# hellojialee/Improved-Body-Parts

Hardware: AMD Instinct MI355X
Metric: fps_512_infer (higher is better)
Workload: dtype bf16; 1 GPU; model=4-stage IMHN @512x512, mode=infer, global_batch=4, input=512, parallelism=dp1

## Files before the change

### improved_body_parts_amd/ops/csrc/bindings.cpp

```cpp
#include <torch/extension.h>

using torch::Tensor;

std::vector<int64_t> bn_v8_geometry(int64_t M, int64_t C);
std::vector<Tensor> bn_stats(const Tensor& x_mc, int64_t C);
std::vector<Tensor> bn_finalize(
    const Tensor& sums, const Tensor& sumsq, int64_t M, const Tensor& gamma,
    const Tensor& beta, const c10::optional<Tensor>& running_mean,
    const c10::optional<Tensor>& running_var,
    const c10::optional<Tensor>& num_batches, double momentum, double eps);
std::vector<Tensor> bn_stats_finalize(
    const Tensor& x_mc, int64_t C, const Tensor& gamma, const Tensor& beta,
    const c10::optional<Tensor>& running_mean,
    const c10::optional<Tensor>& running_var,
    const c10::optional<Tensor>& num_batches, double momentum, double eps);
Tensor bn_act_fwd(const Tensor& x, const Tensor& scale, const Tensor& shift,
                  const c10::optional<Tensor>& residual, double slope, bool act);
std::vector<Tensor> bn_act_bwd(const Tensor& dy, const Tensor& y, const Tensor& x,
                               const c10::optional<Tensor>& mean,
                               const c10::optional<Tensor>& invstd,
                               double slope, bool act, bool need_xhat, int64_t C);
Tensor bn_act_bwd_apply(const Tensor& dpre, const Tensor& x, const Tensor& mean,
                        const Tensor& invstd, const Tensor& gamma,
                        const c10::optional<Tensor>& sum_dpre,
                        const c10::optional<Tensor>& sum_dxhat, int64_t C);

std::vector<Tensor> maxpool2x2_fwd(const Tensor& x, int64_t N, int64_t H,
                                   int64_t W, int64_t C);
Tensor maxpool2x2_bwd(const Tensor& dy, const Tensor& arg, int64_t N, int64_t H,
                      int64_t W, int64_t C);
Tensor upsample2x_fwd(const Tensor& x, int64_t N, int64_t H, int64_t W, int64_t C);
Tensor upsample2x_bwd(const Tensor& dy, int64_t N, int64_t H, int64_t W, int64_t C);
Tensor se_reduce(const Tensor& a, const c10::optional<Tensor>& b, int64_t N,
                 int64_t HW, int64_t C);
Tensor se_scale(const Tensor& x, const Tensor& s, const c10::optional<Tensor>& addc,
                int64_t N, int64_t HW, int64_t C);
Tensor se_gate(const Tensor& pooled, const Tensor& w1, const Tensor& b1,
               const Tensor& w2, const Tensor& b2, double slope,
               double pool_scale);
std::vector<Tensor> se_layer_grouped(const std::vector<Tensor>& xs,
                                     const std::vector<Tensor>& w1s,
                                     const std::vector<Tensor>& b1s,
                                     const std::vector<Tensor>& w2s,
                                     const std::vector<Tensor>& b2s,
                                     double slope);

Tensor focal_l2_fwd(const Tensor& pred, const Tensor& gt, const Tensor& mask,
                    int64_t heat_start, int64_t bkg_start, int64_t gamma,
                    double mtw, double ktw, double alpha, double beta);
Tensor focal_l2_bwd(const Tensor& pred, const Tensor& gt, const Tensor& mask,
                    const Tensor& stack_gscale, int64_t heat_start,
                    int64_t bkg_start, int64_t gamma, double mtw, double ktw,
                    double alpha, double beta);

Tensor conv_mfma_fwd(const Tensor& x, const Tensor& w_packed,
                     const std::vector<int64_t>& geom,
                     const c10::optional<Tensor>& scale,
                     const c10::optional<Tensor>& shift,
                     const c10::optional<Tensor>& residual, bool act,
                     const c10::optional<Tensor>& residual_post,
                     const c10::optional<Tensor>& residual_post2,
                     const c10::optional<Tensor>& x2);

std::vector<Tensor> conv_mfma_fwd_grouped(
    const std::vector<Tensor>& xs, const std::vector<Tensor>& ws_packed,
    const std::vector<std::vector<int64_t>>& geom,
    const std::vector<c10::optional<Tensor>>& scales,
    const std::vector<c10::optional<Tensor>>& shifts,
    const std::vector<c10::optional<Tensor>>& residuals,
    const std::vector<bool>& acts,
    const std::vector<c10::optional<Tensor>>& residual_posts,
    const std::vector<c10::optional<Tensor>>& residual_post2s);

std::vector<int64_t> conv_mfma_tile_plan(int64_t M, int64_t Cout, int64_t K);
std::vector<int64_t> conv_mfma_conv_plan(const Tensor& x,
                                         const Tensor& w_packed,
                                         const std::vector<int64_t>& geom);

void pack_conv_weight(const Tensor& w, Tensor& fwd_pack,
                      const c10::optional<Tensor>& dgrad_pack);

void pack_upfold_weight(const Tensor& w, Tensor& out);
void pack_cat_weight(const Tensor& wa, const Tensor& wb,
                     const c10::optional<Tensor>& scale_a,
                     const c10::optional<Tensor>& scale_b,
                     const c10::optional<Tensor>& shift_a,
                     const c10::optional<Tensor>& shift_b, Tensor& out,
                     Tensor& shift_out);
Tensor conv_mfma_upfold_fwd(const Tensor& x_low, const Tensor& packs,
                            const std::vector<int64_t>& geom,
                            const c10::optional<Tensor>& scale,
                            const c10::optional<Tensor>& shift, bool act,
                            const c10::optional<Tensor>& residual_post,
                            const c10::optional<Tensor>& residual_post2);
std::vector<int64_t> conv_mfma_upfold_plan(int64_t M_low, int64_t Cout,
                                           int64_t Cin);

Tensor conv_mfma_wgrad(const Tensor& x, const Tensor& dy, int64_t N, int64_t H,
                       int64_t W, int64_t Cin, int64_t Cout, int64_t KH,
                       int64_t KW, int64_t stride, int64_t pad_h, int64_t pad_w,
                       int64_t dil_h, int64_t dil_w, int64_t Ho, int64_t Wo);
std::vector<int64_t> conv_wgrad_plan(int64_t M, int64_t Cin, int64_t Cout,
                                     int64_t KH, int64_t KW);
Tensor tr16_probe();

void fused_sgd(const Tensor& chunk_table, double lr, double momentum,
               double weight_decay, int64_t dtype_tag);

Tensor heatmap_gt(const Tensor& joints, const c10::optional<Tensor>& mask_all,
                  const Tensor& limb_pairs, int64_t h, int64_t w,
                  int64_t stride, int64_t heat_start, int64_t bkg_start,
                  int64_t num_layers, double sigma, double paf_sigma,
                  double keypoint_thre, double limb_thre, double paf_thre);

Tensor peaks_batched(const Tensor& maps, int64_t heat_layers, double thre,
                     int64_t radius, int64_t max_peaks);

Tensor limb_scores(const Tensor& paf, const Tensor& peaks, const Tensor& cand_idx,
                   int64_t mid_num, double thre2);
std::vector<Tensor> peaks_canonical(const Tensor& buf, int64_t n_parts);
std::vector<Tensor> limb_match(const Tensor& maps, const Tensor& peaks,
                               const Tensor& offsets, const Tensor& limbs,
                               int64_t first_limb_plane, int64_t mid_num,
                               double thre2, double connect_ration,
                               int64_t max_part);

std::vector<Tensor> people_assemble(const Tensor& peaks, const Tensor& offsets,
                                    const Tensor& rows, const Tensor& counts,
                                    const Tensor& limbs, const Tensor& dt_gt,
                                    double len_rate, double connection_tole,
                                    int64_t remove_recon, int64_t max_people);

void ensemble_merge(const Tensor& src, const Tensor& chan_main,
                    const Tensor& chan_flip, const Tensor& ystart,
                    const Tensor& yw, const Tensor& xstart, const Tensor& xw,
                    Tensor& out, double scale, bool accumulate, int64_t cb,
                    int64_t wr, int64_t wc, int64_t span);

std::vector<Tensor> augment_warp(const Tensor& packed, const Tensor& desc,
                                 int64_t H, int64_t W, int64_t stride,
                                 bool bf16_out);

PYBIND11_MODULE(TORCH_EXTENSION_NAME, m) {
  m.def("bn_v8_geometry", &bn_v8_geometry,
        "debug: [cpb, rpb, rows, grid_y] of the bf16 v8 stats/reduce launch",
        py::arg("M"), py::arg("C"));
  m.def("bn_stats", &bn_stats, "per-channel sum/sumsq of an [M][C] view");
  m.def("bn_finalize", &bn_finalize,
        "mean/invstd/scale/shift epilogue over given (possibly all-reduced) sums");
  m.def("bn_stats_finalize", &bn_stats_finalize,
        "stats + mean/invstd/scale/shift epilogue (+ running-stat update)");
  m.def("bn_act_fwd", &bn_act_fwd, "fused scale/shift (+res) (+leaky)");
  m.def("bn_act_bwd", &bn_act_bwd, "dpre + per-channel reductions");
  m.def("bn_act_bwd_apply", &bn_act_bwd_apply, "BN backward input grad");
  m.def("maxpool2x2_fwd", &maxpool2x2_fwd);
  m.def("maxpool2x2_bwd", &maxpool2x2_bwd);
  m.def("upsample2x_fwd", &upsample2x_fwd);
  m.def("upsample2x_bwd", &upsample2x_bwd);
  m.def("se_reduce", &se_reduce);
  m.def("se_scale", &se_scale);
  m.def("se_gate", &se_gate, "fused GAP-gate: sigmoid(W2@leaky(W1@p+b1)+b2)",
        py::arg("pooled"), py::arg("w1"), py::arg("b1"), py::arg("w2"),
        py::arg("b2"), py::arg("slope"), py::arg("pool_scale") = 1.0);
  m.def("se_layer_grouped", &se_layer_grouped,
        "inference SE layers of independent maps: one launch per stage");
  m.def("focal_l2_fwd", &focal_l2_fwd);
  m.def("focal_l2_bwd", &focal_l2_bwd);
  m.def("conv_mfma_fwd", &conv_mfma_fwd, "MFMA implicit-GEMM conv forward",
        py::arg("x"), py::arg("w_packed"), py::arg("geom"),
        py::arg("scale") = c10::nullopt, py::arg("shift") = c10::nullopt,
        py::arg("residual") = c10::nullopt, py::arg("act") = false,
        py::arg("residual_post") = c10::nullopt,
        py::arg("residual_post2") = c10::nullopt,
        py::arg("x2") = c10::nullopt);
  m.def("conv_mfma_fwd_grouped", &conv_mfma_fwd_grouped,
        "independent MFMA convs in one grouped launch per 8 (+ one combine)",
        py::arg("xs"), py::arg("ws_packed"), py::arg("geom"),
        py::arg("scales"), py::arg("shifts"), py::arg("residuals"),
        py::arg("acts"), py::arg("residual_posts"),
        py::arg("residual_post2s"));
  m.def("conv_mfma_tile_plan", &conv_mfma_tile_plan,
        "debug: [BM, BN, splitk, deep] planned for GEMM extents (M, Cout, K)",
        py::arg("M"), py::arg("Cout"), py::arg("K"));
  m.def("conv_mfma_conv_plan", &conv_mfma_conv_plan,
        "debug: [BM, BN, splitk, deep, gather] planned for conv_mfma_fwd(x, "
        "w_packed, geom); gather 1 = tap-uniform, 0 = generic",
        py::arg("x"), py::arg("w_packed"), py::arg("geom"));
  m.def("pack_conv_weight", &pack_conv_weight,
        "fwd + dgrad weight packs in one kernel",
        py::arg("w"), py::arg("fwd_pack"), py::arg("dgrad_pack") = c10::nullopt);
  m.def("pack_upfold_weight", &pack_upfold_weight,
        "3x3 weight -> four folded 2x2 packs [4][Cout][4*Cin] (nearest-x2 "
        "upsample folded into the conv)",
        py::arg("w"), py::arg("out"));
  m.def("pack_cat_weight", &pack_cat_weight,
        "two 1x1 weights (+ per-channel scales, shifts) -> one [Cout][Ca+Cb] "
        "pack and the fused shift of a two-source 1x1 conv",
        py::arg("wa"), py::arg("wb"), py::arg("scale_a"), py::arg("scale_b"),
        py::arg("shift_a"), py::arg("shift_b"), py::arg("out"),
        py::arg("shift_out"));
  m.def("conv_mfma_upfold_fwd", &conv_mfma_upfold_fwd,
        "conv3x3(nearest_x2(x_low)) + epilogue as four parity 2x2 convs in "
        "one grouped launch",
        py::arg("x_low"), py::arg("packs"), py::arg("geom"),
        py::arg("scale") = c10::nullopt, py::arg("shift") = c10::nullopt,
        py::arg("act") = false, py::arg("residual_post") = c10::nullopt,
        py::arg("residual_post2") = c10::nullopt);
  m.def("conv_mfma_upfold_plan", &conv_mfma_upfold_plan,
        "debug: [BM, BN, splitk, deep] shared by the four parities of an "
        "upfold conv over M_low low-resolution pixels",
        py::arg("M_low"), py::arg("Cout"), py::arg("Cin"));
  m.def("conv_mfma_wgrad", &conv_mfma_wgrad,
        "MFMA implicit-GEMM conv weight gradient (tr16 LDS transpose)");
  m.def("conv_wgrad_plan", &conv_wgrad_plan,
        "debug: [TKD, TCO, waves, elem, kd_cb, chunks, chunk_len, tree group "
        "counts...] planned for a weight gradient with M = N*Ho*Wo",
        py::arg("M"), py::arg("Cin"), py::arg("Cout"), py::arg("KH"),
        py::arg("KW"));
  m.def("tr16_probe", &tr16_probe,
        "debug: ds_read_b64_tr_b16 delivery-map probe");
  m.def("fused_sgd", &fused_sgd);
  m.def("heatmap_gt", &heatmap_gt, "on-device GT heatmap/PAF generation",
        py::arg("joints"), py::arg("mask_all"), py::arg("limb_pairs"),
        py::arg("h"), py::arg("w"), py::arg("stride"), py::arg("heat_start"),
        py::arg("bkg_start"), py::arg("num_layers"), py::arg("sigma"),
        py::arg("paf_sigma"), py::arg("keypoint_thre"), py::arg("limb_thre"),
        py::arg("paf_thre"));
  m.def("limb_scores", &limb_scores);
  m.def("peaks_canonical", &peaks_canonical,
        "peaks_batched buffer -> rows in (channel, y, x) order + channel offsets",
        py::arg("buf"), py::arg("n_parts"));
  m.def("limb_match", &limb_match,
        "per (image, limb): score, filter and greedily match all nA x nB segments",
        py::arg("maps"), py::arg("peaks"), py::arg("offsets"), py::arg("limbs"),
        py::arg("first_limb_plane"), py::arg("mid_num"), py::arg("thre2"),
        py::arg("connect_ration"), py::arg("max_part"));
  m.def("people_assemble", &people_assemble,
        "per image: greedy person assembly over limb_match rows + COCO keypoints",
        py::arg("peaks"), py::arg("offsets"), py::arg("rows"), py::arg("counts"),
        py::arg("limbs"), py::arg("dt_gt"), py::arg("len_rate"),
        py::arg("connection_tole"), py::arg("remove_recon"),
        py::arg("max_people"));
  m.def("peaks_batched", &peaks_batched,
        "fused NMS + centroid refinement over a planar batch, per-image counters",
        py::arg("maps"), py::arg("heat_layers"), py::arg("thre"),
        py::arg("radius"), py::arg("max_peaks"));
  m.def("ensemble_merge", &ensemble_merge,
        "flip-merge + composed bicubic resample of the low-res network output",
        py::arg("src"), py::arg("chan_main"), py::arg("chan_flip"),
        py::arg("ystart"), py::arg("yw"), py::arg("xstart"), py::arg("xw"),
        py::arg("out"), py::arg("scale"), py::arg("accumulate"), py::arg("cb"),
        py::arg("wr"), py::arg("wc"), py::arg("span"));
  m.def("augment_warp", &augment_warp,
        "batched affine warp of ragged uint8 records -> [image NHWC, "
        "mask_miss, mask_all on the stride grid]",
        py::arg("packed"), py::arg("desc"), py::arg("H"), py::arg("W"),
        py::arg("stride"), py::arg("bf16_out"));
}
```

### improved_body_parts_amd/ops/csrc/conv_mfma.hip

```cpp
#include <torch/extension.h>
#include <ATen/hip/HIPContext.h>
#include <algorithm>
#include <type_traits>
#include <vector>
#include "common.h"
#include "conv_params.h"
#include "conv_plan.h"

namespace ibp {

typedef short short8 __attribute__((ext_vector_type(8)));
typedef float floatx4 __attribute__((ext_vector_type(4)));
typedef float floatx2 __attribute__((ext_vector_type(2)));
typedef unsigned short ushortv8 __attribute__((ext_vector_type(8)));
typedef unsigned short ushortv4 __attribute__((ext_vector_type(4)));

__device__ __forceinline__ int lds_off(int row, int k) {
  return row * BK + (k ^ ((row & 7) << 3));
}

template <int BM, int BN, bool DEEP, bool UP, bool CAT, bool TU,
          typename Params>
__device__ __forceinline__ void conv_mfma_body(const Params& p,
                                               const int bid,
                                               unsigned short* lds_a,
                                               unsigned short* lds_b) {
  const int tid = threadIdx.x;
  const int lane = tid & 63;
  const int wave = tid >> 6;

  const int ntiles_n = (p.Cout + BN - 1) / BN;
  const int sk = bid % p.splitk;
  const int tile = bid / p.splitk;
  const int mt = tile / ntiles_n;
  const int nt = tile % ntiles_n;
  const long long m0 = (long long)mt * BM;
  const int n0 = nt * BN;

  constexpr int WROWS = (BM == 128) ? ((BN == 128) ? 2 : 4) : 2;
  constexpr int WCOLS = 4 / WROWS;
  constexpr int WM = BM / WROWS;
  constexpr int WN = BN / WCOLS;
  constexpr int AFRAG = WM / 16;
  constexpr int BFRAG = WN / 16;
  const int wm = (WCOLS == 1) ? wave : (wave >> 1);
  const int wn = (WCOLS == 1) ? 0 : (wave & 1);
  const int row_base = wm * WM;
  const int col_base = wn * WN;

  floatx4 acc[AFRAG][BFRAG];
  #pragma unroll
  for (int i = 0; i < AFRAG; ++i)
    #pragma unroll
    for (int j = 0; j < BFRAG; ++j) acc[i][j] = floatx4{0.f, 0.f, 0.f, 0.f};

  constexpr int A_ELEMS = BM * BK / 256;
  constexpr int B_ELEMS = BN * BK / 256;
  constexpr int TPR_A = BK / A_ELEMS;
  constexpr int TPR_B = BK / B_ELEMS;
  const int a_row = tid / TPR_A;
  const int a_off = (tid % TPR_A) * A_ELEMS;
  const int b_row = tid / TPR_B;
  const int b_off = (tid % TPR_B) * B_ELEMS;

  const long long a_m = m0 + a_row;
  int a_n = 0, a_ho = 0, a_wo = 0;
  bool a_valid_row = a_m < p.M;
  if (a_valid_row && p.m32) {
    unsigned t = (unsigned)a_m;
    a_wo = (int)(t % (unsigned)p.Wo); t /= (unsigned)p.Wo;
    a_ho = (int)(t % (unsigned)p.Ho);
    a_n = (int)(t / (unsigned)p.Ho);
  } else if (a_valid_row) {
    long long t = a_m;
    a_wo = (int)(t % p.Wo); t /= p.Wo;
    a_ho = (int)(t % p.Ho);
    a_n = (int)(t / p.Ho);
  }
  const int hi_base = a_ho * p.stride - p.pad_h;
  const int wi_base = a_wo * p.stride - p.pad_w;

  const int nk_total = (p.K + BK - 1) / BK;
  const int nk_chunk = (nk_total + p.splitk - 1) / p.splitk;
  const int k_begin = sk * nk_chunk;
  const int nk = min(nk_chunk, nk_total - k_begin);
  if (nk <= 0) return;

  unsigned short a_reg0[A_ELEMS];
  unsigned short b_reg0[B_ELEMS];
  unsigned short a_reg1[A_ELEMS];
  unsigned short b_reg1[B_ELEMS];

  int t_kk = k_begin * BK + a_off;
  int t_ci = 0, t_kh = 0, t_kw = 0;
  if constexpr (!CAT) {
    const int t_f = t_kk / p.Cin;
    t_ci = t_kk - t_f * p.Cin;
    t_kh = t_f / p.KW;
    t_kw = t_f - t_kh * p.KW;
  }
  auto tap_advance = [&](int& ci, int& kh, int& kw, int step) {
// ... 409 lines not shown
      }
      #pragma unroll
      for (int i = 0; i < AFRAG; ++i) {
        const long long m = m0 + row_base + i * 16 + epix;
        if (m >= p.M) continue;
        const long long lin = m * p.Cout + col;
        if (p.splitk > 1) {
          *reinterpret_cast<floatx4*>(ws_slice + lin) = acc[i][j];
          continue;
        }
        const long long idx = out_idx(i, col, lin);
        *reinterpret_cast<ushortv4*>(p.y + idx) =
            finish(acc[i][j], idx, sc, sh);
      }
      continue;
    }
    if (p.pair_epi) {
      #pragma unroll
      for (int r = 0; r < 4; r += 2) {
        if (col + r >= p.Cout) continue;
        const float sc0 = p.scale ? p.scale[col + r] : 1.f;
        const float sc1 = p.scale ? p.scale[col + r + 1] : 1.f;
        const float sh0 = p.shift ? p.shift[col + r] : 0.f;
        const float sh1 = p.shift ? p.shift[col + r + 1] : 0.f;
        #pragma unroll
        for (int i = 0; i < AFRAG; ++i) {
          const long long m = m0 + row_base + i * 16 + epix;
          if (m >= p.M) continue;
          const long long lin = m * p.Cout + col + r;
          if (p.splitk > 1) {
            *reinterpret_cast<floatx2*>(ws_slice + lin) =
                floatx2{acc[i][j][r], acc[i][j][r + 1]};
            continue;
          }
          const long long idx = out_idx(i, col + r, lin);
          unsigned r0 = 0, r1 = 0, r2 = 0;
          if (p.res) r0 = *reinterpret_cast<const unsigned*>(p.res + idx);
          if (p.res_post)
            r1 = *reinterpret_cast<const unsigned*>(p.res_post + idx);
          if (p.res_post2)
            r2 = *reinterpret_cast<const unsigned*>(p.res_post2 + idx);
          float v0 = acc[i][j][r] * sc0 + sh0;
          float v1 = acc[i][j][r + 1] * sc1 + sh1;
          if (p.res) {
            v0 += us2f((unsigned short)r0); v1 += us2f((unsigned short)(r0 >> 16));
          }
          if (p.act) { v0 = leaky(v0, 0.01f); v1 = leaky(v1, 0.01f); }
          if (p.res_post) {
            v0 += us2f((unsigned short)r1); v1 += us2f((unsigned short)(r1 >> 16));
          }
          if (p.res_post2) {
            v0 += us2f((unsigned short)r2); v1 += us2f((unsigned short)(r2 >> 16));
          }
          *reinterpret_cast<unsigned*>(p.y + idx) =
              (unsigned)f2us(v0) | ((unsigned)f2us(v1) << 16);
        }
      }
      continue;
    }
    #pragma unroll
    for (int r = 0; r < 4; ++r) {
      if (col + r >= p.Cout) continue;
      const float sc = p.scale ? p.scale[col + r] : 1.f;
      const float sh = p.shift ? p.shift[col + r] : 0.f;
      #pragma unroll
      for (int i = 0; i < AFRAG; ++i) {
        const long long m = m0 + row_base + i * 16 + epix;
        if (m >= p.M) continue;
        const long long lin = m * p.Cout + col + r;
        if (p.splitk > 1) {
          ws_slice[lin] = acc[i][j][r];
          continue;
        }
        const long long idx = out_idx(i, col + r, lin);
        float v = acc[i][j][r] * sc + sh;
        if (p.res) v += us2f(p.res[idx]);
        if (p.act) v = leaky(v, 0.01f);
        if (p.res_post) v += us2f(p.res_post[idx]);
        if (p.res_post2) v += us2f(p.res_post2[idx]);
        p.y[idx] = f2us(v);
      }
    }
  }
}

template <int BM, int BN, bool DEEP = false, bool CAT = false, bool TU = false>
__global__ __launch_bounds__(256, 2) void conv_mfma_kernel(ConvParams p) {
  static_assert(!(CAT && TU), "the two-source conv keeps its own gather");
  __shared__ unsigned short lds_a[2 * BM * BK];
  __shared__ unsigned short lds_b[2 * BN * BK];
  conv_mfma_body<BM, BN, DEEP, false, CAT, TU>(p, blockIdx.x, lds_a, lds_b);
}

template <bool UP>
__global__ __launch_bounds__(256, 2) void conv_mfma_grouped_kernel(
    ConvGroupParams g) {
  __shared__ __attribute__((aligned(16))) unsigned short lds[4 * 128 * BK];
  const int gb = blockIdx.x;
  int pi = 0, base = 0, cfg = g.cfg[0];
  #pragma unroll
  for (int i = 0; i < kMaxGroup - 1; ++i) {
    if (i + 1 < g.n && gb >= g.block_end[i]) {
      pi = i + 1;
      base = g.block_end[i];
      cfg = g.cfg[i + 1];
    }
  }
  typedef __attribute__((address_space(4))) const char* kernarg_bytes;
  kernarg_bytes ka = (kernarg_bytes)__builtin_amdgcn_kernarg_segment_ptr();
  typedef __attribute__((address_space(4))) const ConvParams* kernarg_params;
  const auto& p = *(kernarg_params)(ka + offsetof(ConvGroupParams, p) +
                                    (size_t)pi * sizeof(ConvParams));
  const int bid = gb - base;
  #define IBP_BODY(BM_, BN_, DEEP_, TU_)                                     \
    conv_mfma_body<BM_, BN_, DEEP_, UP, false, TU_>(p, bid, lds,            \
                                                    lds + 2 * BM_ * BK)
  switch (cfg | (p.gather ? 8 : 0)) {
    case tile_cfg(128, 128, false): IBP_BODY(128, 128, false, false); break;
    case tile_cfg(128, 128, true): IBP_BODY(128, 128, true, false); break;
    case tile_cfg(128, 64, false): IBP_BODY(128, 64, false, false); break;
    case tile_cfg(128, 64, true): IBP_BODY(128, 64, true, false); break;
    case tile_cfg(64, 64, false): IBP_BODY(64, 64, false, false); break;
    case tile_cfg(64, 64, true): IBP_BODY(64, 64, true, false); break;
    case tile_cfg(32, 64, false): IBP_BODY(32, 64, false, false); break;
    case tile_cfg(32, 64, true): IBP_BODY(32, 64, true, false); break;
    case 8 | tile_cfg(128, 128, false): IBP_BODY(128, 128, false, true); break;
    case 8 | tile_cfg(128, 128, true): IBP_BODY(128, 128, true, true); break;
    case 8 | tile_cfg(128, 64, false): IBP_BODY(128, 64, false, true); break;
    case 8 | tile_cfg(128, 64, true): IBP_BODY(128, 64, true, true); break;
    case 8 | tile_cfg(64, 64, false): IBP_BODY(64, 64, false, true); break;
    case 8 | tile_cfg(64, 64, true): IBP_BODY(64, 64, true, true); break;
    case 8 | tile_cfg(32, 64, false): IBP_BODY(32, 64, false, true); break;
    default: IBP_BODY(32, 64, true, true); break;
  }
  #undef IBP_BODY
}

static_assert(std::is_same<decltype(&conv_mfma_grouped_kernel<false>),
                           void (*)(ConvGroupParams)>::value &&
                  std::is_same<decltype(&conv_mfma_grouped_kernel<true>),
                               void (*)(ConvGroupParams)>::value,
              "conv_mfma_grouped_kernel must take the table as its only "
              "argument: it is read at kernarg offset 0");

__device__ __forceinline__ float combine_one(float v, float sc, float sh,
                                             bool has_scale, bool has_res,
                                             float r0, int act, bool has_rp,
                                             float r1, bool has_rp2, float r2) {
  if (has_scale) v = v * sc + sh;
  if (has_res) v += r0;
  if (act) v = leaky(v, 0.01f);
  if (has_rp) v += r1;
  if (has_rp2) v += r2;
  return v;
}

__device__ __forceinline__ long long scatter_pixel(unsigned m,
                                                   const OutScatter& s) {
  const unsigned j = m % (unsigned)s.Wo; m /= (unsigned)s.Wo;
  const unsigned i = m % (unsigned)s.Ho;
  const unsigned n = m / (unsigned)s.Ho;
  return ((long long)n * (2 * s.Ho) + 2 * i + s.py) * (2 * s.Wo) + 2 * j + s.px;
}

template <bool VEC, bool UP>
__device__ __forceinline__ void splitk_combine_body(
    const float* __restrict__ ws, unsigned short* __restrict__ y,
    const float* __restrict__ scale, const float* __restrict__ shift,
    const unsigned short* __restrict__ res,
    const unsigned short* __restrict__ res_post,
    const unsigned short* __restrict__ res_post2, long long total, int C,
    int act, int splitk, int bid, int nblocks, const OutScatter& os) {
  if constexpr (VEC) {
    const int C8 = C >> 3;
    const long long groups = total >> 3;
    const long long step = (long long)nblocks * blockDim.x;
    long long g = bid * (long long)blockDim.x + threadIdx.x;
    if (g >= groups) return;
    int c8 = (int)(g % C8);
    const int cstep = (int)(step % C8);
    unsigned row = UP ? (unsigned)(g / C8) : 0u;
    const unsigned rstep = UP ? (unsigned)(step / C8) : 0u;
    for (; g < groups; g += step) {
      const long long w = g << 3;
      const long long i = UP ? scatter_pixel(row, os) * C + c8 * 8 : w;
      floatx4 lo = floatx4{0.f, 0.f, 0.f, 0.f}, hi = lo;
      for (int s = 0; s < splitk; ++s) {
        const float* src = ws + (long long)s * total + w;
        lo += *reinterpret_cast<const floatx4*>(src);
        hi += *reinterpret_cast<const floatx4*>(src + 4);
      }
      floatx4 sc_lo = lo, sc_hi = lo, sh_lo = lo, sh_hi = lo;
      if (scale) {
        sc_lo = *reinterpret_cast<const floatx4*>(scale + c8 * 8);
        sc_hi = *reinterpret_cast<const floatx4*>(scale + c8 * 8 + 4);
        sh_lo = *reinterpret_cast<const floatx4*>(shift + c8 * 8);
        sh_hi = *reinterpret_cast<const floatx4*>(shift + c8 * 8 + 4);
      }
      ushortv8 r0 = ushortv8{0, 0, 0, 0, 0, 0, 0, 0}, r1 = r0, r2 = r0;
      if (res) r0 = *reinterpret_cast<const ushortv8*>(res + i);
      if (res_post) r1 = *reinterpret_cast<const ushortv8*>(res_post + i);
      if (res_post2) r2 = *reinterpret_cast<const ushortv8*>(res_post2 + i);
      ushortv8 out;
      #pragma unroll
      for (int e = 0; e < 4; ++e) {
        out[e] = f2us(combine_one(lo[e], sc_lo[e], sh_lo[e], scale != nullptr,
                                  res != nullptr, us2f(r0[e]), act,
                                  res_post != nullptr, us2f(r1[e]),
                                  res_post2 != nullptr, us2f(r2[e])));
        out[e + 4] = f2us(combine_one(
            hi[e], sc_hi[e], sh_hi[e], scale != nullptr, res != nullptr,
            us2f(r0[e + 4]), act, res_post != nullptr, us2f(r1[e + 4]),
            res_post2 != nullptr, us2f(r2[e + 4])));
      }
      *reinterpret_cast<ushortv8*>(y + i) = out;
      c8 += cstep;
      if (c8 >= C8) c8 -= C8;
      if constexpr (UP) {
        row += rstep;
        if (c8 < cstep) ++row;
      }
    }
  } else {
    for (long long w = bid * (long long)blockDim.x + threadIdx.x;
         w < total; w += (long long)nblocks * blockDim.x) {
      int c = (int)(w % C);
      const long long i =
          UP ? scatter_pixel((unsigned)(w / C), os) * C + c : w;
      float v = 0.f;
      for (int s = 0; s < splitk; ++s) v += ws[(long long)s * total + w];
      v = combine_one(v, scale ? scale[c] : 1.f, scale ? shift[c] : 0.f,
                      scale != nullptr, res != nullptr,
                      res ? us2f(res[i]) : 0.f, act, res_post != nullptr,
                      res_post ? us2f(res_post[i]) : 0.f,
                      res_post2 != nullptr,
                      res_post2 ? us2f(res_post2[i]) : 0.f);
      y[i] = f2us(v);
    }
// ... 207 lines not shown
                         const OptTensor& residual_post2) {
  TORCH_CHECK(x.is_cuda() && x.scalar_type() == at::ScalarType::BFloat16,
              "conv_mfma: x must be a bf16 device tensor");
  TORCH_CHECK(w_packed.is_contiguous(), "conv_mfma: pack must be contiguous");
  TORCH_CHECK(geom.size() == 15, "conv_mfma: geom needs 15 ints");
  ConvProblem q;
  ibp::ConvParams& p = q.p;
  int* const row[15] = {&p.N, &p.H, &p.W, &p.Cin, &p.Cout, &p.KH, &p.KW,
                        &p.stride, &p.pad_h, &p.pad_w, &p.dil_h, &p.dil_w,
                        &p.Ho, &p.Wo, &p.zs};
  for (int i = 0; i < 15; ++i) *row[i] = (int)geom[i];
  p.x = reinterpret_cast<const unsigned short*>(x.data_ptr());
  p.w = reinterpret_cast<const unsigned short*>(w_packed.data_ptr());
  p.scale = scale.has_value() ? scale->data_ptr<float>() : nullptr;
  p.shift = shift.has_value() ? shift->data_ptr<float>() : nullptr;
  p.res = bf16_ptr(residual);
  p.res_post = bf16_ptr(residual_post);
  p.res_post2 = bf16_ptr(residual_post2);
  p.act = act ? 1 : 0;
  return q;
}

void set_second_source(ConvProblem& q, const Tensor& x, const Tensor& x2,
                       const Tensor& w_packed) {
  ibp::ConvParams& p = q.p;
  TORCH_CHECK(x2.is_cuda() && x2.device() == x.device() &&
              x2.scalar_type() == at::ScalarType::BFloat16 && x2.dim() == 4 &&
              x2.is_contiguous(at::MemoryFormat::ChannelsLast) &&
              x2.size(0) == p.N && x2.size(2) == p.H && x2.size(3) == p.W,
              "conv_mfma: x2 must be channels_last bf16 [N, Cin2, H, W]");
  TORCH_CHECK(x.dim() == 4 &&
              x.is_contiguous(at::MemoryFormat::ChannelsLast) &&
              x.size(0) == p.N && x.size(1) == p.Cin && x.size(2) == p.H &&
              x.size(3) == p.W,
              "conv_mfma: with x2, x must be channels_last [N, Cin, H, W]");
  p.Cin2 = (int)x2.size(1);
  p.x2 = reinterpret_cast<const unsigned short*>(x2.data_ptr());
  TORCH_CHECK(w_packed.numel() == (int64_t)p.Cout * (p.Cin + p.Cin2),
              "conv_mfma: two-source pack must be [Cout][Cin + Cin2]");
}

Tensor alloc_output(ConvProblem& q, const Tensor& x) {
  Tensor y = torch::empty({q.p.N, q.p.Ho, q.p.Wo, q.p.Cout}, x.options());
  q.p.y = reinterpret_cast<unsigned short*>(y.data_ptr());
  return y;
}

template <class F>
void with_flag(bool flag, F&& f) {
  if (flag) f(std::true_type{});
  else f(std::false_type{});
}

template <class F>
void with_tile(const ConvPlan& plan, F&& f) {
  using i128 = std::integral_constant<int, 128>;
  using i64 = std::integral_constant<int, 64>;
  using i32 = std::integral_constant<int, 32>;
  with_flag(plan.t.deep, [&](auto deep) {
    if (plan.t.BM == 128 && plan.t.BN == 128) f(i128{}, i128{}, deep);
    else if (plan.t.BM == 128) f(i128{}, i64{}, deep);
    else if (plan.t.BM == 64) f(i64{}, i64{}, deep);
    else f(i32{}, i64{}, deep);
  });
}

void launch_single(const ConvPlan& plan, hipStream_t stream) {
  const ibp::ConvParams& p = plan.p;
  TORCH_CHECK(!p.up, "upfold plans launch through the grouped kernel");
  with_tile(plan, [&](auto bm, auto bn, auto deep) {
    TORCH_CHECK(!(p.Cin2 != 0 && p.gather != 0));
    with_flag(p.Cin2 != 0, [&](auto cat) {
      with_flag(p.gather != 0, [&](auto tu) {
        if constexpr (!(decltype(cat)::value && decltype(tu)::value))
          hipLaunchKernelGGL(
              (ibp::conv_mfma_kernel<decltype(bm)::value, decltype(bn)::value,
                                     decltype(deep)::value,
                                     decltype(cat)::value,
                                     decltype(tu)::value>),
              dim3(plan.nblocks), dim3(256), 0, stream, p);
      });
    });
  });
  if (p.splitk > 1)
    with_flag(plan.vec_combine, [&](auto vec) {
      hipLaunchKernelGGL(ibp::splitk_combine_kernel<decltype(vec)::value>,
                         dim3(ibp::combine_blocks(plan)), dim3(256), 0, stream,
                         p.ws, p.y, p.scale, p.shift, p.res, p.res_post,
                         p.res_post2, (long long)p.M * p.Cout, p.Cout, p.act,
                         p.splitk);
    });
}

void launch_group(const ibp::GroupPlan& gp, hipStream_t stream) {
  with_flag(gp.up, [&](auto up) {
    hipLaunchKernelGGL(ibp::conv_mfma_grouped_kernel<decltype(up)::value>,
                       dim3(gp.blocks), dim3(256), 0, stream, gp.g);
    if (gp.cg.n > 0)
      hipLaunchKernelGGL(
          ibp::splitk_combine_grouped_kernel<decltype(up)::value>,
          dim3(gp.cblocks), dim3(256), 0, stream, gp.cg);
  });
}

void run_plans(std::vector<ConvPlan>& plans, hipStream_t stream,
               const at::TensorOptions& f32) {
  std::vector<Tensor> keep;
  auto workspace = [&](long long elems) -> float* {
    if (elems <= 0) return nullptr;
    keep.push_back(torch::empty({elems}, f32));
    return keep.back().data_ptr<float>();
  };
  for (size_t first = 0; first < plans.size(); first += ibp::kMaxGroup) {
    const size_t last =
        std::min(plans.size(), first + (size_t)ibp::kMaxGroup);
    ConvPlan& head = plans[first];
    if (last - first == 1 && !head.p.up) {
      if (head.ws_elems > 0) ibp::set_workspace(head, workspace(head.ws_elems));
      launch_single(head, stream);
    } else {
      float* ws = workspace(ibp::group_workspace(plans, first, last));
      launch_group(ibp::assemble_group(plans, first, last, ws), stream);
    }
  }
}

}

Tensor conv_mfma_fwd(const Tensor& x, const Tensor& w_packed,
                     const std::vector<int64_t>& geom, const OptTensor& scale,
                     const OptTensor& shift, const OptTensor& residual,
                     bool act, const OptTensor& residual_post,
                     const OptTensor& residual_post2, const OptTensor& x2) {
  ConvProblem q = make_problem(x, w_packed, geom, scale, shift, residual, act,
                               residual_post, residual_post2);
  if (x2.has_value()) set_second_source(q, x, *x2, w_packed);
  Tensor y = alloc_output(q, x);
  std::vector<ConvPlan> plans{ibp::plan_conv(q)};
  run_plans(plans, at::hip::getCurrentHIPStream().stream(),
            x.options().dtype(torch::kFloat32));
  return y;
}

std::vector<Tensor> conv_mfma_fwd_grouped(
    const std::vector<Tensor>& xs, const std::vector<Tensor>& ws_packed,
    const std::vector<std::vector<int64_t>>& geom,
    const std::vector<OptTensor>& scales, const std::vector<OptTensor>& shifts,
    const std::vector<OptTensor>& residuals, const std::vector<bool>& acts,
    const std::vector<OptTensor>& residual_posts,
    const std::vector<OptTensor>& residual_post2s) {
  const size_t n = xs.size();
  TORCH_CHECK(n > 0 && ws_packed.size() == n && geom.size() == n &&
              scales.size() == n && shifts.size() == n &&
              residuals.size() == n && acts.size() == n &&
              residual_posts.size() == n && residual_post2s.size() == n,
              "conv_mfma_fwd_grouped: argument lists differ in length");
  std::vector<ConvPlan> plans;
  std::vector<Tensor> ys;
  plans.reserve(n);
  ys.reserve(n);
  for (size_t i = 0; i < n; ++i) {
    TORCH_CHECK(xs[i].device() == xs[0].device());
    ConvProblem q = make_problem(xs[i], ws_packed[i], geom[i], scales[i],
                                 shifts[i], residuals[i], acts[i],
                                 residual_posts[i], residual_post2s[i]);
    ys.push_back(alloc_output(q, xs[i]));
    plans.push_back(ibp::plan_conv(q));
  }
  run_plans(plans, at::hip::getCurrentHIPStream().stream(),
            xs[0].options().dtype(torch::kFloat32));
  return ys;
}

Tensor conv_mfma_upfold_fwd(const Tensor& x_low, const Tensor& packs,
                            const std::vector<int64_t>& geom,
                            const OptTensor& scale, const OptTensor& shift,
                            bool act, const OptTensor& residual_post,
                            const OptTensor& residual_post2) {
  ConvProblem q = make_problem(x_low, packs, geom, scale, shift, c10::nullopt,
                               act, residual_post, residual_post2);
  ibp::ConvParams& p = q.p;
  const int64_t N = p.N, H = p.H, W = p.W, Cin = p.Cin, Cout = p.Cout;
  TORCH_CHECK(p.KH == 3 && p.KW == 3 && p.stride == 1 && p.pad_h == 1 &&
              p.pad_w == 1 && p.dil_h == 1 && p.dil_w == 1 && p.zs == 1 &&
              p.Ho == 2 * H && p.Wo == 2 * W,
              "conv_mfma_upfold_fwd: geom must be a 3x3 stride-1 pad-1 conv "
              "with Ho x Wo = 2H x 2W");
  TORCH_CHECK(x_low.is_contiguous() && x_low.numel() == N * H * W * Cin,
              "conv_mfma_upfold_fwd: x_low must be contiguous [N][H][W][Cin]");
  TORCH_CHECK(packs.is_cuda() &&
              packs.scalar_type() == at::ScalarType::BFloat16 &&
              packs.numel() == 16 * Cout * Cin,
              "conv_mfma_upfold_fwd: packs must be bf16 [4][Cout][4*Cin]");
  for (const auto* r : {&residual_post, &residual_post2})
    TORCH_CHECK(!r->has_value() || (*r)->numel() == 4 * N * H * W * Cout,
                "conv_mfma_upfold_fwd: residuals must be bf16 "
                "[N][2H][2W][Cout]");
  Tensor y = alloc_output(q, x_low);
  p.KH = p.KW = 2;
  p.Ho = p.H;
  p.Wo = p.W;
  p.up = 1;
  q.tile = ibp::plan_upfold_tile(N * H * W, p.Cout, p.Cin);
  std::vector<ConvPlan> plans;
  plans.reserve(4);
  for (int par = 0; par < 4; ++par) {
    p.py = par >> 1;
    p.px = par & 1;
    p.pad_h = 1 - p.py;
    p.pad_w = 1 - p.px;
    p.w = reinterpret_cast<const unsigned short*>(packs.data_ptr()) +
          (long long)par * Cout * 4 * Cin;
    plans.push_back(ibp::plan_conv(q));
  }
  run_plans(plans, at::hip::getCurrentHIPStream().stream(),
            x_low.options().dtype(torch::kFloat32));
  return y;
}

std::vector<int64_t> conv_mfma_tile_plan(int64_t M, int64_t Cout, int64_t K) {
  const ibp::TilePlan t = ibp::plan_tile(M, (int)Cout, (int)K);
  return {t.BM, t.BN, t.splitk, t.deep ? 1 : 0};
}

std::vector<int64_t> conv_mfma_conv_plan(const Tensor& x,
                                         const Tensor& w_packed,
                                         const std::vector<int64_t>& geom) {
  const ConvProblem q =
      make_problem(x, w_packed, geom, c10::nullopt, c10::nullopt, c10::nullopt,
                   false, c10::nullopt, c10::nullopt);
  const ConvPlan plan = ibp::plan_conv(q);
  return {plan.t.BM, plan.t.BN, plan.p.splitk, plan.t.deep ? 1 : 0,
          plan.p.gather};
}

std::vector<int64_t> conv_mfma_upfold_plan(int64_t M_low, int64_t Cout,
                                           int64_t Cin) {
  const ibp::TilePlan t = ibp::plan_upfold_tile(M_low, (int)Cout, (int)Cin);
  return {t.BM, t.BN, t.splitk, t.deep ? 1 : 0};
}
```

### improved_body_parts_amd/ops/csrc/conv_params.h

```cpp
#pragma once

#include <cstddef>
#include <type_traits>

namespace ibp {

constexpr int BK = 64;

struct ConvParams {
  const unsigned short* x;
  const unsigned short* w;
  unsigned short* y;
  const float* scale;
  const float* shift;
  const unsigned short* res;
  const unsigned short* res_post;
  const unsigned short* res_post2;
  int N, H, W, Cin, Cout, KH, KW;
  int stride, pad_h, pad_w, dil_h, dil_w, Ho, Wo;
  int zs;
  long long M;
  int K;
  int n_mtiles;
  int act;
  int splitk;
  float* ws;
  int vec_epi;
  int pair_epi;
  int m32;
  int up, py, px;
  int Cin2;
  const unsigned short* x2;
  int gather;
};

constexpr long long kGatherMaxBytes = 0x7fffffffLL;
constexpr unsigned kGatherOob = 0x80000000u;

constexpr int kMaxGroup = 8;

struct ConvGroupParams {
  ConvParams p[kMaxGroup];
  int block_end[kMaxGroup];
  int cfg[kMaxGroup];
  int n;
};

constexpr int tile_cfg(int BM, int BN, bool deep) {
  return ((BM == 128 ? (BN == 128 ? 0 : 1) : (BM == 64 ? 2 : 3)) << 1) |
         (deep ? 1 : 0);
}

static_assert(offsetof(ConvGroupParams, p) == 0 &&
                  std::is_standard_layout<ConvGroupParams>::value &&
                  std::is_trivially_copyable<ConvGroupParams>::value &&
                  sizeof(ConvParams) % alignof(ConvParams) == 0 &&
                  sizeof(ConvGroupParams) <= 4096,
              "ConvGroupParams layout: problem array first, within the "
              "kernel-argument limit");

struct OutScatter {
  int up, py, px, Ho, Wo;
};

struct CombineProblem {
  const float* ws;
  unsigned short* y;
  const float* scale;
  const float* shift;
  const unsigned short* res;
  const unsigned short* res_post;
  const unsigned short* res_post2;
  long long total;
  int C, act, splitk, vec;
  OutScatter os;
};

struct CombineGroupParams {
  CombineProblem c[kMaxGroup];
  int block_end[kMaxGroup];
  int n;
};

}
```

### improved_body_parts_amd/ops/csrc/conv_plan.h

```cpp
#pragma once

#include <algorithm>
#include <cstdint>
#include <cstdlib>
#include <optional>
#include <stdexcept>
#include <string>
#include <vector>

#include "conv_params.h"

namespace ibp {

struct TilePlan {
  int BM, BN, n_mtiles, ntiles, splitk, nk_block;
  bool deep;
};

struct ConvProblem {
  ConvParams p{};
  std::optional<TilePlan> tile;
};

struct ConvPlan {
// ... 128 lines not shown
  plan.p.ws = ws;
  plan.vec_combine = plan.vec_combine && !misaligned(ws, 16);
}

inline int combine_blocks(const ConvPlan& plan) {
  const long long total = plan.p.M * plan.p.Cout;
  const long long work = plan.vec_combine ? total / 8 : total;
  const long long g = (work + 255) / 256;
  return (int)(g < 4096 ? (g > 0 ? g : 1) : 4096);
}

inline long long ws_slice(const ConvPlan& plan) {
  return (plan.ws_elems + 3) / 4 * 4;
}
inline long long group_workspace(const std::vector<ConvPlan>& plans,
                                 size_t first, size_t last) {
  long long total = 0;
  for (size_t i = first; i < last; ++i) total += ws_slice(plans[i]);
  return total;
}

struct GroupPlan {
  int order[kMaxGroup];
  long long ws_off[kMaxGroup];
  ConvGroupParams g;
  CombineGroupParams cg;
  int blocks, cblocks;
  bool up;
};

inline GroupPlan assemble_group(std::vector<ConvPlan>& plans, size_t first,
                                size_t last, float* ws_base) {
  const int n = (int)(last - first);
  if (n < 1 || n > kMaxGroup || last > plans.size())
    throw std::invalid_argument("grouped conv: 1 to kMaxGroup members");
  GroupPlan gp{};
  gp.up = plans[first].p.up != 0;
  long long ws_total = 0;
  for (int i = 0; i < n; ++i) {
    ConvPlan& plan = plans[first + i];
    if ((plan.p.up != 0) != gp.up)
      throw std::invalid_argument(
          "grouped conv: upfold and plain members cannot mix");
    if (plan.p.Cin2 != 0)
      throw std::invalid_argument(
          "grouped conv: a two-source conv launches on its own");
    gp.order[i] = i;
    gp.ws_off[i] = ws_total;
    if (plan.ws_elems > 0) set_workspace(plan, ws_base + ws_total);
    ws_total += ws_slice(plan);
  }
  std::stable_sort(gp.order, gp.order + n, [&](int a, int b) {
    return plans[first + a].t.nk_block > plans[first + b].t.nk_block;
  });
  for (int i = 0; i < kMaxGroup; ++i) {
    const ConvPlan& plan = plans[first + gp.order[i < n ? i : n - 1]];
    if (i < n) gp.blocks += plan.nblocks;
    gp.g.p[i] = plan.p;
    gp.g.cfg[i] = tile_cfg(plan.t.BM, plan.t.BN, plan.t.deep);
    gp.g.block_end[i] = gp.blocks;
  }
  gp.g.n = n;
  int nc = 0;
  for (int i = 0; i < n; ++i) {
    const ConvPlan& plan = plans[first + gp.order[i]];
    if (plan.p.splitk <= 1) continue;
    const ConvParams& p = plan.p;
    gp.cblocks += combine_blocks(plan);
    gp.cg.c[nc] = CombineProblem{p.ws, p.y, p.scale, p.shift, p.res,
                                 p.res_post, p.res_post2,
                                 (long long)p.M * p.Cout, p.Cout, p.act,
                                 p.splitk, plan.vec_combine ? 1 : 0,
                                 OutScatter{p.up, p.py, p.px, p.Ho, p.Wo}};
    gp.cg.block_end[nc++] = gp.cblocks;
  }
  for (int i = nc; i < kMaxGroup; ++i) {
    gp.cg.c[i] = gp.cg.c[nc > 0 ? nc - 1 : 0];
    gp.cg.block_end[i] = gp.cblocks;
  }
  gp.cg.n = nc;
  return gp;
}

}
```

Baseline: 571.5 images/s.

## Fuse split-K reduction into conv kernel via last-arriving-block tickets

Split-K conv tiles now take an atomic ticket per output tile, and the last block to arrive sums every partial slice from the workspace and applies the epilogue (scale/shift, residuals, leaky activation) in place. This removes the separate combine kernel launch and its extra pass over the workspace. Per-stream counter buffers are allocated lazily and are reset by the last block. The cost is that the final block of each tile does serial reduction work, plus atomics, fences and extra register pressure in the main kernel. The path is on by default and can be turned off with IBP_SPLITK_FUSE=0.

```diff
diff --git a/improved_body_parts_amd/ops/csrc/bindings.cpp b/improved_body_parts_amd/ops/csrc/bindings.cpp
--- a/improved_body_parts_amd/ops/csrc/bindings.cpp
+++ b/improved_body_parts_amd/ops/csrc/bindings.cpp
@@ -76,6 +76,10 @@
 std::vector<int64_t> conv_mfma_conv_plan(const Tensor& x,
                                          const Tensor& w_packed,
                                          const std::vector<int64_t>& geom);
+Tensor conv_mfma_splitk_counters();
+std::vector<int64_t> conv_mfma_fuse_plan(const std::vector<int64_t>& Ms,
+                                         const std::vector<int64_t>& Couts,
+                                         const std::vector<int64_t>& Ks);
 
 void pack_conv_weight(const Tensor& w, Tensor& fwd_pack,
                       const c10::optional<Tensor>& dgrad_pack);
@@ -186,6 +190,13 @@
         "debug: [BM, BN, splitk, deep, gather] planned for conv_mfma_fwd(x, "
         "w_packed, geom); gather 1 = tap-uniform, 0 = generic",
         py::arg("x"), py::arg("w_packed"), py::arg("geom"));
+  m.def("conv_mfma_splitk_counters", &conv_mfma_splitk_counters,
+        "debug: int32 view of the current stream's arrival counters of the "
+        "fused split-K ending; all zero between launches");
+  m.def("conv_mfma_fuse_plan", &conv_mfma_fuse_plan,
+        "debug: per member of a grouped launch over GEMM extents (M, Cout, "
+        "K), 1 if it takes the fused split-K ending",
+        py::arg("Ms"), py::arg("Couts"), py::arg("Ks"));
   m.def("pack_conv_weight", &pack_conv_weight,
         "fwd + dgrad weight packs in one kernel",
         py::arg("w"), py::arg("fwd_pack"), py::arg("dgrad_pack") = c10::nullopt);
diff --git a/improved_body_parts_amd/ops/csrc/conv_mfma.hip b/improved_body_parts_amd/ops/csrc/conv_mfma.hip
--- a/improved_body_parts_amd/ops/csrc/conv_mfma.hip
+++ b/improved_body_parts_amd/ops/csrc/conv_mfma.hip
@@ -1,6 +1,9 @@
 #include <torch/extension.h>
 #include <ATen/hip/HIPContext.h>
 #include <algorithm>
+#include <functional>
+#include <map>
+#include <mutex>
 #include <type_traits>
 #include <vector>
 #include "common.h"
@@ -17,6 +20,18 @@
 
 __device__ __forceinline__ int lds_off(int row, int k) {
   return row * BK + (k ^ ((row & 7) << 3));
+}
+
+__device__ __forceinline__ float combine_one(float v, float sc, float sh,
+                                             bool has_scale, bool has_res,
+                                             float r0, int act, bool has_rp,
+                                             float r1, bool has_rp2, float r2) {
+  if (has_scale) v = v * sc + sh;
+  if (has_res) v += r0;
+  if (act) v = leaky(v, 0.01f);
+  if (has_rp) v += r1;
+  if (has_rp2) v += r2;
+  return v;
 }
 
 template <int BM, int BN, bool DEEP, bool UP, bool CAT, bool TU,
@@ -592,6 +607,159 @@
       }
     }
   }
+
+  if (p.splitk > 1 && p.fuse) {
+    asm volatile("s_waitcnt vmcnt(0)" ::: "memory");
+    __syncthreads();
+    volatile int* const ticket = reinterpret_cast<volatile int*>(lds_a);
+    if (tid == 0) {
+      __builtin_amdgcn_fence(__ATOMIC_RELEASE, "agent");
+      asm volatile("s_waitcnt vmcnt(0)" ::: "memory");
+      const int t = __hip_atomic_fetch_add(p.cnt + tile, 1, __ATOMIC_RELAXED,
+                                           __HIP_MEMORY_SCOPE_AGENT);
+      if (t == p.splitk - 1)
+        __hip_atomic_store(p.cnt + tile, 0, __ATOMIC_RELAXED,
+                           __HIP_MEMORY_SCOPE_AGENT);
+      *ticket = t;
+    }
+    __syncthreads();
+    if (*ticket != p.splitk - 1) return;
+    if (tid == 0) __builtin_amdgcn_fence(__ATOMIC_ACQUIRE, "agent");
+    asm volatile("s_waitcnt vmcnt(0)" ::: "memory");
+    __syncthreads();
+
+    const long long slab = p.M * p.Cout;
+    #pragma unroll
+    for (int i = 0; i < AFRAG; ++i)
+      #pragma unroll
+      for (int j = 0; j < BFRAG; ++j) acc[i][j] = floatx4{0.f, 0.f, 0.f, 0.f};
+    if (p.vec_epi) {
+      constexpr int SU = (AFRAG * BFRAG >= 8) ? 1 : 8 / (AFRAG * BFRAG);
+      for (int s0 = 0; s0 < p.splitk; s0 += SU) {
+        #pragma unroll
+        for (int u = 0; u < SU; ++u) {
+          const bool live = SU == 1 || s0 + u < p.splitk;
+          const float* src = p.ws + (long long)(live ? s0 + u : 0) * slab;
+          #pragma unroll
+          for (int i = 0; i < AFRAG; ++i)
+            #pragma unroll
+            for (int j = 0; j < BFRAG; ++j) {
+              const long long m = m0 + row_base + i * 16 + epix;
+              const int col = n0 + col_base + j * 16 + ech4;
+              const bool ok = m < p.M && col < p.Cout;
+              const unsigned off =
+                  ok ? ((unsigned)m * (unsigned)p.Cout + (unsigned)col) * 4u
+                     : 0u;
+              const floatx4 v = *reinterpret_cast<const floatx4*>(
+                  reinterpret_cast<const char*>(src) + off);
+              acc[i][j] += live ? v : floatx4{0.f, 0.f, 0.f, 0.f};
+            }
+        }
+      }
+    } else {
+      #pragma unroll
+      for (int i = 0; i < AFRAG; ++i)
+        #pragma unroll
+        for (int j = 0; j < BFRAG; ++j)
+          #pragma unroll
+          for (int r = 0; r < 4; ++r) {
+            const long long m = m0 + row_base + i * 16 + epix;
+            const int col = n0 + col_base + j * 16 + ech4 + r;
+            const bool ok = m < p.M && col < p.Cout;
+            const float* src = p.ws + (ok ? m * p.Cout + col : 0LL);
+            float v = 0.f;
+            for (int s = 0; s < p.splitk; ++s) v += src[(long long)s * slab];
+            acc[i][j][r] = v;
+          }
+    }
+
+    const bool has_scale = p.scale != nullptr, has_res = p.res != nullptr;
+    const bool has_rp = p.res_post != nullptr;
+    const bool has_rp2 = p.res_post2 != nullptr;
+    #pragma unroll
+    for (int j = 0; j < BFRAG; ++j) {
+      const int col = n0 + col_base + j * 16 + ech4;
+      if (col >= p.Cout) continue;
+      if (p.fuse == 2) {
+        floatx4 sc = floatx4{1.f, 1.f, 1.f, 1.f};
+        floatx4 sh = floatx4{0.f, 0.f, 0.f, 0.f};
+        if (has_scale) {
+          sc = *reinterpret_cast<const floatx4*>(p.scale + col);
+          sh = *reinterpret_cast<const floatx4*>(p.shift + col);
+        }
+        #pragma unroll
+        for (int i = 0; i < AFRAG; ++i) {
+          const long long m = m0 + row_base + i * 16 + epix;
+          if (m >= p.M) continue;
+          const long long idx = out_idx(i, col, m * p.Cout + col);
+          ushortv4 r0 = ushortv4{0, 0, 0, 0}, r1 = r0, r2 = r0;
+          if (has_res) r0 = *reinterpret_cast<const ushortv4*>(p.res + idx);
+          if (has_rp) r1 = *reinterpret_cast<const ushortv4*>(p.res_post + idx);
+          if (has_rp2)
+            r2 = *reinterpret_cast<const ushortv4*>(p.res_post2 + idx);
+          ushortv4 out;
+          #pragma unroll
+          for (int r = 0; r < 4; ++r)
+            out[r] = f2us(combine_one(acc[i][j][r], sc[r], sh[r], has_scale,
+                                      has_res, us2f(r0[r]), p.act, has_rp,
+                                      us2f(r1[r]), has_rp2, us2f(r2[r])));
+          *reinterpret_cast<ushortv4*>(p.y + idx) = out;
+        }
+        continue;
+      }
+      if (p.pair_epi) {
+        #pragma unroll
+        for (int r = 0; r < 4; r += 2) {
+          if (col + r >= p.Cout) continue;
+          const float sc0 = has_scale ? p.scale[col + r] : 1.f;
+          const float sc1 = has_scale ? p.scale[col + r + 1] : 1.f;
+          const float sh0 = has_scale ? p.shift[col + r] : 0.f;
+          const float sh1 = has_scale ? p.shift[col + r + 1] : 0.f;
+          #pragma unroll
+          for (int i = 0; i < AFRAG; ++i) {
+            const long long m = m0 + row_base + i * 16 + epix;
+            if (m >= p.M) continue;
+            const long long idx = out_idx(i, col + r, m * p.Cout + col + r);
+            unsigned r0 = 0, r1 = 0, r2 = 0;
+            if (has_res) r0 = *reinterpret_cast<const unsigned*>(p.res + idx);
+            if (has_rp)
+              r1 = *reinterpret_cast<const unsigned*>(p.res_post + idx);
+            if (has_rp2)
+              r2 = *reinterpret_cast<const unsigned*>(p.res_post2 + idx);
+            const float v0 = combine_one(
+                acc[i][j][r], sc0, sh0, has_scale, has_res,
+                us2f((unsigned short)r0), p.act, has_rp,
+                us2f((unsigned short)r1), has_rp2, us2f((unsigned short)r2));
+            const float v1 = combine_one(
+                acc[i][j][r + 1], sc1, sh1, has_scale, has_res,
+                us2f((unsigned short)(r0 >> 16)), p.act, has_rp,
+                us2f((unsigned short)(r1 >> 16)), has_rp2,
+                us2f((unsigned short)(r2 >> 16)));
+            *reinterpret_cast<unsigned*>(p.y + idx) =
+                (unsigned)f2us(v0) | ((unsigned)f2us(v1) << 16);
+          }
+        }
+        continue;
+      }
+      #pragma unroll
+      for (int r = 0; r < 4; ++r) {
+        if (col + r >= p.Cout) continue;
+        const float sc = has_scale ? p.scale[col + r] : 1.f;
+        const float sh = has_scale ? p.shift[col + r] : 0.f;
+        #pragma unroll
+        for (int i = 0; i < AFRAG; ++i) {
+          const long long m = m0 + row_base + i * 16 + epix;
+          if (m >= p.M) continue;
+          const long long idx = out_idx(i, col + r, m * p.Cout + col + r);
+          p.y[idx] = f2us(combine_one(
+              acc[i][j][r], sc, sh, has_scale, has_res,
+              has_res ? us2f(p.res[idx]) : 0.f, p.act, has_rp,
+              has_rp ? us2f(p.res_post[idx]) : 0.f, has_rp2,
+              has_rp2 ? us2f(p.res_post2[idx]) : 0.f));
+        }
+      }
+    }
+  }
 }
 
 template <int BM, int BN, bool DEEP = false, bool CAT = false, bool TU = false>
@@ -652,18 +820,6 @@
                                void (*)(ConvGroupParams)>::value,
               "conv_mfma_grouped_kernel must take the table as its only "
               "argument: it is read at kernarg offset 0");
-
-__device__ __forceinline__ float combine_one(float v, float sc, float sh,
-                                             bool has_scale, bool has_res,
-                                             float r0, int act, bool has_rp,
-                                             float r1, bool has_rp2, float r2) {
-  if (has_scale) v = v * sc + sh;
-  if (has_res) v += r0;
-  if (act) v = leaky(v, 0.01f);
-  if (has_rp) v += r1;
-  if (has_rp2) v += r2;
-  return v;
-}
 
 __device__ __forceinline__ long long scatter_pixel(unsigned m,
                                                    const OutScatter& s) {
@@ -1037,7 +1193,7 @@
       });
     });
   });
-  if (p.splitk > 1)
+  if (p.splitk > 1 && !p.fuse)
     with_flag(plan.vec_combine, [&](auto vec) {
       hipLaunchKernelGGL(ibp::splitk_combine_kernel<decltype(vec)::value>,
                          dim3(ibp::combine_blocks(plan)), dim3(256), 0, stream,
@@ -1058,8 +1214,50 @@
   });
 }
 
+#define IBP_HIP_OK(call)                                                    \
+  do {                                                                      \
+    const hipError_t ibp_err_ = (call);                                     \
+    TORCH_CHECK(ibp_err_ == hipSuccess, #call ": ",                         \
+                hipGetErrorString(ibp_err_));                               \
+  } while (0)
+
+struct CounterKey {
+  int device;
+  hipStream_t stream;
+  bool operator<(const CounterKey& o) const {
+    return device != o.device ? device < o.device
+                              : std::less<hipStream_t>()(stream, o.stream);
+  }
+};
+
+int* splitk_counters(hipStream_t stream) {
+  static std::mutex mu;
+  static std::map<CounterKey, int*> bufs;
+  int device = 0;
+  IBP_HIP_OK(hipGetDevice(&device));
+  std::lock_guard<std::mutex> lock(mu);
+  auto it = bufs.find(CounterKey{device, stream});
+  if (it != bufs.end()) return it->second;
+  hipStreamCaptureStatus cap = hipStreamCaptureStatusNone;
+  IBP_HIP_OK(hipStreamIsCapturing(stream, &cap));
+  if (cap != hipStreamCaptureStatusNone) return nullptr;
+  int* buf = nullptr;
+  IBP_HIP_OK(hipMalloc(&buf, ibp::kFuseCounters * sizeof(int)));
+  IBP_HIP_OK(
+      hipMemsetAsync(buf, 0, ibp::kFuseCounters * sizeof(int), stream));
+  bufs.emplace(CounterKey{device, stream}, buf);
+  return buf;
+}
+
 void run_plans(std::vector<ConvPlan>& plans, hipStream_t stream,
                const at::TensorOptions& f32) {
+  int* cnt = nullptr;
+  if (ibp::fuse_enabled())
+    for (const ConvPlan& plan : plans)
+      if (plan.p.splitk > 1) {
+        cnt = splitk_counters(stream);
+        break;
+      }
   std::vector<Tensor> keep;
   auto workspace = [&](long long elems) -> float* {
     if (elems <= 0) return nullptr;
@@ -1070,12 +1268,16 @@
     const size_t last =
         std::min(plans.size(), first + (size_t)ibp::kMaxGroup);
     ConvPlan& head = plans[first];
+    ibp::assign_counters(plans, first, last, cnt,
+                         cnt ? ibp::kFuseCounters : 0);
     if (last - first == 1 && !head.p.up) {
       if (head.ws_elems > 0) ibp::set_workspace(head, workspace(head.ws_elems));
       launch_single(head, stream);
     } else {
       float* ws = workspace(ibp::group_workspace(plans, first, last));
-      launch_group(ibp::assemble_group(plans, first, last, ws), stream);
+      ibp::GroupPlan gp = ibp::assemble_group(plans, first, last, ws);
+      ibp::drop_fused(gp);
+      launch_group(gp, stream);
     }
   }
 }
@@ -1194,3 +1396,36 @@
   const ibp::TilePlan t = ibp::plan_upfold_tile(M_low, (int)Cout, (int)Cin);
   return {t.BM, t.BN, t.splitk, t.deep ? 1 : 0};
 }
+
+Tensor conv_mfma_splitk_counters() {
+  int* buf = splitk_counters(at::hip::getCurrentHIPStream().stream());
+  TORCH_CHECK(buf != nullptr,
+              "conv_mfma_splitk_counters: no buffer yet and the stream is "
+              "capturing");
+  int device = 0;
+  IBP_HIP_OK(hipGetDevice(&device));
+  return torch::from_blob(
+      buf, {ibp::kFuseCounters},
+      torch::TensorOptions().dtype(torch::kInt32).device(torch::kCUDA, device));
+}
+
+std::vector<int64_t> conv_mfma_fuse_plan(const std::vector<int64_t>& Ms,
+                                         const std::vector<int64_t>& Couts,
+                                         const std::vector<int64_t>& Ks) {
+  TORCH_CHECK(Ms.size() == Couts.size() && Ms.size() == Ks.size() &&
+              Ms.size() <= (size_t)ibp::kMaxGroup);
+  std::vector<ConvPlan> plans(Ms.size());
+  for (size_t i = 0; i < Ms.size(); ++i) {
+    plans[i].t = ibp::plan_tile(Ms[i], (int)Couts[i], (int)Ks[i]);
+    plans[i].p = ibp::ConvParams{};
+    plans[i].p.M = Ms[i];
+    plans[i].p.Cout = (int)Couts[i];
+    plans[i].p.K = (int)Ks[i];
+    plans[i].p.splitk = plans[i].t.splitk;
+  }
+  static int dummy[ibp::kFuseCounters];
+  ibp::assign_counters(plans, 0, plans.size(), dummy, ibp::kFuseCounters);
+  std::vector<int64_t> out;
+  for (const ConvPlan& plan : plans) out.push_back(plan.p.fuse ? 1 : 0);
+  return out;
+}
diff --git a/improved_body_parts_amd/ops/csrc/conv_params.h b/improved_body_parts_amd/ops/csrc/conv_params.h
--- a/improved_body_parts_amd/ops/csrc/conv_params.h
+++ b/improved_body_parts_amd/ops/csrc/conv_params.h
@@ -32,7 +32,11 @@
   int Cin2;
   const unsigned short* x2;
   int gather;
+  int fuse;
+  int* cnt;
 };
+
+constexpr int kFuseCounters = 4096;
 
 constexpr long long kGatherMaxBytes = 0x7fffffffLL;
 constexpr unsigned kGatherOob = 0x80000000u;
diff --git a/improved_body_parts_amd/ops/csrc/conv_plan.h b/improved_body_parts_amd/ops/csrc/conv_plan.h
--- a/improved_body_parts_amd/ops/csrc/conv_plan.h
+++ b/improved_body_parts_amd/ops/csrc/conv_plan.h
@@ -234,4 +234,72 @@
   return gp;
 }
 
-}
+
+inline bool fuse_enabled() {
+  if (const char* e = getenv("IBP_SPLITK_FUSE"))
+    if (e[0] == '0' && e[1] == '\0') return false;
+  return true;
+}
+
+inline bool fuse_eligible(const ConvPlan& plan, long long cnt_used,
+                          long long cnt_capacity) {
+  if (plan.p.splitk <= 1 || !fuse_enabled()) return false;
+  const int nk_total = (plan.p.K + BK - 1) / BK;
+  const int nk_chunk = (nk_total + plan.p.splitk - 1) / plan.p.splitk;
+  if ((long long)(plan.p.splitk - 1) * nk_chunk >= nk_total) return false;
+  if (4LL * plan.p.M * plan.p.Cout > kGatherMaxBytes) return false;
+  return cnt_used + plan.t.ntiles <= cnt_capacity;
+}
+
+inline void set_counters(ConvPlan& plan, int* cnt) {
+  ConvParams& p = plan.p;
+  p.cnt = cnt;
+  p.fuse = 0;
+  if (cnt == nullptr) return;
+  const bool wide =
+      p.Cout % 4 == 0 &&
+      !(misaligned(p.scale, 16) || misaligned(p.shift, 16) ||
+        misaligned(p.res, 8) || misaligned(p.res_post, 8) ||
+        misaligned(p.res_post2, 8) || misaligned(p.y, 8));
+  p.fuse = wide ? 2 : 1;
+}
+
+inline long long assign_counters(std::vector<ConvPlan>& plans, size_t first,
+                                 size_t last, int* cnt_base,
+                                 long long capacity) {
+  long long used = 0;
+  for (size_t i = first; i < last; ++i) {
+    ConvPlan& plan = plans[i];
+    if (cnt_base != nullptr && fuse_eligible(plan, used, capacity)) {
+      set_counters(plan, cnt_base + used);
+      used += plan.t.ntiles;
+    } else {
+      set_counters(plan, nullptr);
+    }
+  }
+  return used;
+}
+
+inline void drop_fused(GroupPlan& gp) {
+  CombineGroupParams out{};
+  int nc = 0, k = 0, blocks = 0;
+  for (int i = 0; i < gp.g.n; ++i) {
+    if (gp.g.p[i].splitk <= 1) continue;
+    const int own = gp.cg.block_end[k] - (k > 0 ? gp.cg.block_end[k - 1] : 0);
+    if (gp.g.p[i].fuse == 0) {
+      blocks += own;
+      out.c[nc] = gp.cg.c[k];
+      out.block_end[nc++] = blocks;
+    }
+    ++k;
+  }
+  for (int i = nc; i < kMaxGroup; ++i) {
+    out.c[i] = nc > 0 ? out.c[nc - 1] : gp.cg.c[0];
+    out.block_end[i] = blocks;
+  }
+  out.n = nc;
+  gp.cg = out;
+  gp.cblocks = blocks;
+}
+
+}
```

Measured after the change: 472.9 images/s. -17.3%, worse.
